# tuanad121/Python-WORLD

Measured on AMD Instinct MI355X. Metric: analysis+synthesis frames/sec (and xRT), 16 kHz / 5 ms hop, higher is better.
Workload: dtype f64; 1 GPU; BASELINE config 2 per GPU: 64 x 10 s synthetic 16 kHz utterances, DIO+StoneMask+CheapTrick+D4C encode + pulse-wise synthesis decode with on-device Philox noise (not the reference-parity host-noise path), HBM-resident; utterances_per_gpu=64, distinct_utterances=64, fs=16000, lanes_per_gpu=1

## Files before the change

include/world_hip.h:

```cpp
#ifndef WORLD_HIP_H
#define WORLD_HIP_H
#include <stddef.h>
#include <stdint.h>

#ifdef __cplusplus
extern "C" {
#endif

typedef struct wh_ctx wh_ctx;
typedef struct wh_batch wh_batch;

int wh_version(void);
const char* wh_last_error(void);

int wh_device_count(int* count);
int wh_ctx_create(int device, wh_ctx** out);
int wh_ctx_destroy(wh_ctx* ctx);
int wh_ctx_trim(wh_ctx* ctx);
int wh_malloc(void** dptr, size_t bytes);
int wh_free(void* dptr);
int wh_memcpy_h2d(void* dst, const void* h_src, size_t bytes, void* stream);
int wh_memcpy_d2h(void* h_dst, const void* src, size_t bytes, void* stream);
int wh_memset(void* dst, int value, size_t bytes, void* stream);
int wh_stream_sync(void* stream);
int wh_host_alloc(void** h_ptr, size_t bytes);
int wh_host_free(void* h_ptr);
int wh_copy_mapped(wh_ctx* ctx, void* stream, void* dst, const void* src, size_t bytes, int max_blocks);

#define WH_FLAG_STONEMASK_WINDOW 0
#define WH_FLAG_EVENT_OVERFLOW 1
#define WH_FLAG_NOISE_SHORT 2
#define WH_FLAG_NO_PULSE 3
#define WH_FLAG_PULSE_OVERFLOW 4
#define WH_FLAG_OOB 5
int wh_take_flags(wh_ctx* ctx, void* stream, int32_t* h_flags16);
int wh_bounds_build(void);
int wh_bounds_last(int64_t* out4);
int wh_bounds_selftest(wh_ctx* ctx, void* stream);
int wh_math_probe(wh_ctx* ctx, void* stream, int which, const double* in, double* out, int64_t n);
int wh_fft_probe(wh_ctx* ctx, void* stream, int n, int gt, int snt, int inverse, const double* in, double* out, int64_t count);
int wh_flags_post(wh_ctx* ctx, void* stream, int discard);
int wh_flags_poll(wh_ctx* ctx, int32_t* h_flags16);

int wh_profile_enable(wh_ctx* ctx, int on);
int wh_profile_collect(wh_ctx* ctx, char* names, size_t names_bytes, float* ms, int max_records, int* n_records);

int wh_batch_create(wh_ctx* ctx, int n_utt, const int64_t* h_x_off, const int64_t* h_frame_off, wh_batch** out);
int wh_batch_destroy(wh_batch* b);
int64_t wh_num_frames(int64_t n_samples, double fs, double frame_period_ms);

int wh_cheaptrick(wh_ctx* ctx, void* stream, const wh_batch* b, const double* x, const double* tp, double* f0,
                  const double* vuv, double fs, int fft_size, double q1, double* spectrogram, double* ps_spectrogram);

int wh_d4c(wh_ctx* ctx, void* stream, const wh_batch* b, const double* x, const double* tp, double* f0,
           const double* vuv, double fs, double threshold, int fft_size_for_spectrum, double* aperiodicity,
           double* coarse_ap);
int wh_d4c_bands(double fs, int requiem);

int wh_d4c_requiem(wh_ctx* ctx, void* stream, const wh_batch* b, const double* x, const double* tp, double* f0,
                   const double* vuv, double fs, double threshold, int fft_size, double* band_aperiodicity);

int wh_dio(wh_ctx* ctx, void* stream, const wh_batch* b, const double* x, const double* tp, double fs, double f0_floor,
           double f0_ceil, double target_fs, double frame_period_ms, double allowed_range, int n_bands,
           const double* h_band_f0, const int32_t* h_band_bias, const int32_t* h_band_len, const double* h_band_taps,
           const double* h_lowcut, int lowcut_half, double* f0_out, double* vuv_out, double* cand_out, double* raw_out);

int wh_harvest(wh_ctx* ctx, void* stream, const wh_batch* b, const double* x, const double* tp, double fs,
               double f0_floor, double f0_ceil, double frame_period_ms, int decimation_ratio, const double* h_ba,
               const double* h_zi, int n_bands, const double* h_band_f0, const int32_t* h_band_half,
               const double* h_band_taps, double* f0_out, double* vuv_out, double* dbg_y, double* dbg_raw,
               double* dbg_f0_1ms);
int wh_harvest_set_event_caps(wh_ctx* ctx, const int64_t* h_caps, int64_t n);
int wh_harvest_event_counts(wh_ctx* ctx, void* stream, int64_t* h_caps_out, int64_t n);
// ... 72 lines not shown
```

python-world_amd/csrc/wh_api.hip:

```cpp
#include <math.h>
#include <string.h>

#include "wh_device.h"
#include "wh_host.h"
#include "wh_math.h"

namespace {
thread_local std::string g_last_error;

__global__ void frame_utt_kernel(const int64_t* __restrict__ frame_off, int n_utt, int64_t total, int32_t* __restrict__ out) {
  int64_t i = (int64_t)blockIdx.x * blockDim.x + threadIdx.x;
  const int64_t stride = (int64_t)gridDim.x * blockDim.x;
  for (; i < total; i += stride) {
    int lo = 0, hi = n_utt;
    while (hi - lo > 1) {
      int mid = (lo + hi) >> 1;
      if (frame_off[mid] <= i) lo = mid; else hi = mid;
    }
    out[i] = lo;
  }
}

__global__ void copy_mapped_kernel(double2* __restrict__ dst, const double2* __restrict__ src, size_t n16, double* dst_tail,
                                   const double* src_tail) {
// ... 87 lines not shown
  e.host.assign(reinterpret_cast<const char*>(host), reinterpret_cast<const char*>(host) + bytes);
  *dptr = e.d;
  return 0;
}
int persistent_scratch(wh_ctx* ctx, const std::string& slot, size_t bytes, void** dptr) {
  wh_ctx::Persist& e = ctx->persist[slot];
  if (e.cap < bytes || !e.d) {
    if (e.d) {
      WH_CHECK(hipDeviceSynchronize());
      WH_CHECK(hipFree(e.d));
      e.d = nullptr;
    }
    const size_t want = bytes < 256 ? 256 : bytes + bytes / 4;
    WH_CHECK(hipMalloc(&e.d, want));
    e.cap = want;
  }
  *dptr = e.d;
  return 0;
}
}

static std::vector<int (*)(unsigned long long*)>& bounds_readers() {
  static std::vector<int (*)(unsigned long long*)> v;
  return v;
}
int wh::bounds_register(int (*reader)(unsigned long long*)) {
  bounds_readers().push_back(reader);
  return (int)bounds_readers().size();
}
static thread_local int64_t g_bounds_last[4] = {0, 0, 0, 0};

extern "C" {

int wh_version(void) { return 108; }
const char* wh_last_error(void) { return g_last_error.c_str(); }

int wh_device_count(int* count) {
  WH_CHECK(hipGetDeviceCount(count));
  return 0;
}

int wh_ctx_create(int device, wh_ctx** out) {
  if (!out) return wh::fail_msg("wh_ctx_create", "null out pointer");
  WH_CHECK(hipSetDevice(device));
  wh_ctx* c = new wh_ctx();
  c->device = device;
  std::vector<double2> tw(WH_TWIDDLE_ENTRIES);
  tw[0] = tw[1] = make_double2(1.0, 0.0);
  for (int n = 2; n <= WH_MAX_TWIDDLE; n <<= 1) {
    for (int k = 0; k < n; ++k) {
      long double a = -2.0L * 3.14159265358979323846264338327950288L * (long double)k / (long double)n;
      tw[n + k] = make_double2((double)cosl(a), (double)sinl(a));
    }
    tw[n] = make_double2(1.0, 0.0);
    if (n >= 2) tw[n + n / 2] = make_double2(-1.0, 0.0);
    if (n >= 4) {
      tw[n + n / 4] = make_double2(0.0, -1.0);
      tw[n + 3 * n / 4] = make_double2(0.0, 1.0);
    }
  }
  for (int R = 2; R <= 8; R <<= 1)
    for (int m = R; m <= WH_MAX_FFT; m <<= 1)
      for (int k = 0; k < m / R; ++k)
        for (int r = 1; r < R; ++r) tw[wh::fft_ptw_offset(m, R) + k * (R - 1) + r - 1] = tw[m + k * r];
  hipError_t e = hipMalloc((void**)&c->d_twiddle, tw.size() * sizeof(double2));
  if (e == hipSuccess) e = hipMemcpy(c->d_twiddle, tw.data(), tw.size() * sizeof(double2), hipMemcpyHostToDevice);
  if (e == hipSuccess) e = hipMalloc((void**)&c->d_flags, 16 * sizeof(int32_t));
// ... 114 lines not shown
  constexpr int N = 512;
  extern __shared__ __attribute__((aligned(16))) char smem[];
  const int g = threadIdx.x / GT, t = threadIdx.x % GT;
  const long long b = (long long)blockIdx.x * (SNT / GT) + g;
  const wh::ckp<double2> lds = wh::ck_make(reinterpret_cast<double2*>(smem), (long long)N * (SNT / GT), wh::WH_CK_LDS_OTHER);
  const wh::ckp<double2> s = wh::ck_sub(lds, (long long)g * N, N, wh::WH_CK_LDS_MAIN);
  const wh::ckp<const double2> tw = wh::ck_make(tw_base, WH_TWIDDLE_ENTRIES, wh::WH_CK_TWIDDLE);
  for (int i = t; i < N; i += GT) s[i] = b < count ? in[b * N + i] : make_double2(0.0, 0.0);
  __syncthreads();
  if (inv) wh::fft_lds_wave<N, true, GT, SNT>(s, tw + N);
  else wh::fft_lds_wave<N, false, GT, SNT>(s, tw + N);
  if (b < count)
    for (int i = t; i < N; i += GT) out[b * N + i] = s[i];
}
}
int wh_fft_probe(wh_ctx* ctx, void* stream, int n, int gt, int snt, int inverse, const double* in, double* out, int64_t count) {
  if (!ctx || !in || !out || count < 0 || n != 512 || (inverse != 0 && inverse != 1))
    return wh::fail_msg("wh_fft_probe", "bad argument");
  WH_ENTER(ctx);
  if (count == 0) return 0;
  const hipStream_t st = (hipStream_t)stream;
  const double2* a = reinterpret_cast<const double2*>(in);
  double2* o = reinterpret_cast<double2*>(out);
  auto launch = [&](auto kernel, int g, int t) {
    const int per = t / g;
    hipLaunchKernelGGL(kernel, dim3((unsigned)((count + per - 1) / per)), dim3(t), sizeof(double2) * 512 * per, st, a, o,
                       (const double2*)ctx->d_twiddle, (long long)count, inverse);
  };
  if (gt == 64 && snt == 64) launch(fft_probe_kernel<64, 64>, 64, 64);
  else if (gt == 128 && snt == 256) launch(fft_probe_kernel<128, 256>, 128, 256);
  else if (gt == 256 && snt == 256) launch(fft_probe_kernel<256, 256>, 256, 256);
  else return wh::fail_msg("wh_fft_probe", "shape not built (gt, snt): (64, 64), (128, 256), (256, 256)");
  WH_LAUNCH_CHECK("fft_probe_kernel");
  return 0;
}

int wh_bounds_last(int64_t* out4) {
  if (!out4) return wh::fail_msg("wh_bounds_last", "null argument");
  for (int i = 0; i < 4; ++i) out4[i] = g_bounds_last[i];
  return 0;
}

int wh_take_flags(wh_ctx* ctx, void* stream, int32_t* h_flags16) {
  if (!ctx || !h_flags16) return wh::fail_msg("wh_take_flags", "null argument");
  WH_ENTER(ctx);
  hipStream_t st = (hipStream_t)stream;
  WH_CHECK(hipMemcpyAsync(h_flags16, ctx->d_flags, 16 * sizeof(int32_t), hipMemcpyDeviceToHost, st));
  WH_CHECK(hipMemsetAsync(ctx->d_flags, 0, 16 * sizeof(int32_t), st));
  WH_CHECK(hipStreamSynchronize(st));
  drain_posted(ctx, h_flags16, true);
  for (int i = 0; i < 4; ++i) g_bounds_last[i] = 0;
  if (!bounds_readers().empty()) {
    WH_CHECK(hipDeviceSynchronize());
    for (auto rd : bounds_readers()) {
      unsigned long long rec[4] = {0, 0, 0, 0};
      if (rd(rec)) return wh::fail_msg("wh_take_flags", "reading a bounds record failed");
      if (rec[0]) {
        if (!g_bounds_last[0]) for (int i = 1; i < 4; ++i) g_bounds_last[i] = (int64_t)rec[i];
        g_bounds_last[0] += (int64_t)rec[0];
      }
    }
    if (g_bounds_last[0]) h_flags16[WH_FLAG_OOB] = 1;
  }
  return 0;
}

// ... 169 lines not shown
```

python-world_amd/csrc/wh_d4c.hip:

```cpp
#include <map>

#include <hip/hip_runtime.h>
#ifndef WH_D4C_PAIR
#define WH_D4C_PAIR 1
#endif
#ifndef WH_D4C_HOIST
#define WH_D4C_HOIST 0
#endif
#ifndef WH_D4C_PAIR_MINW
#define WH_D4C_PAIR_MINW 2
#endif
__device__ __forceinline__ int wh_opaque_tid() {
  int t = threadIdx.x;
#if !WH_D4C_HOIST
  asm volatile("" : "+v"(t));
#endif
  return t;
}
#define WH_TID wh_opaque_tid()
#include "wh_host.h"
#include "wh_spectral.h"

#ifndef WH_D4C_ABLATE
#define WH_D4C_ABLATE 0
#endif
#ifndef WH_D4C_KEEP_W
#define WH_D4C_KEEP_W 4
#endif
#ifndef WH_D4C_GATHER_UNCOND
#define WH_D4C_GATHER_UNCOND 1
#endif
#ifndef WH_D4C_REGFED
#define WH_D4C_REGFED 1
#endif
#ifndef WH_D4C_RMAXR
#define WH_D4C_RMAXR 0
#endif
#ifndef WH_D4C_MAXR
#define WH_D4C_MAXR 0
#endif
constexpr int d4c_maxr(int n) { return WH_D4C_MAXR ? WH_D4C_MAXR : ((n <= 1024 || WH_D4C_REGFED) ? 8 : 4); }
constexpr int d4c_rmaxr(int n) { return WH_D4C_RMAXR ? WH_D4C_RMAXR : ((n <= 1024 || WH_D4C_REGFED) ? 8 : 4); }
#ifndef WH_LOVE_REGWIN
#define WH_LOVE_REGWIN 1
#endif
#ifndef WH_LOVE_MAXR
#define WH_LOVE_MAXR 8
#endif
#ifndef WH_D4C_MINBLK
#define WH_D4C_MINBLK 4
#endif
#ifndef WH_D4C_WIN_UNROLL
#define WH_D4C_WIN_UNROLL 4
#endif
#ifndef WH_D4C_CENT_LOOP
#define WH_D4C_CENT_LOOP 0
#endif
#ifdef WH_D4C_STAGE_TIMER
__device__ unsigned long long g_d4c_stage[16];
__device__ unsigned long long g_d4c_t0[1 << 20];
#define STAGE_TIMER_BEGIN { if (threadIdx.x == 0) g_d4c_t0[blockIdx.x & ((1 << 20) - 1)] = __builtin_readcyclecounter(); }
#define STAGE_MARK(i) { __syncthreads(); if (threadIdx.x == 0) { const unsigned long long _t = __builtin_readcyclecounter(); atomicAdd(&g_d4c_stage[i], _t - g_d4c_t0[blockIdx.x & ((1 << 20) - 1)]); g_d4c_t0[blockIdx.x & ((1 << 20) - 1)] = _t; } }
#else
#define STAGE_TIMER_BEGIN
#define STAGE_MARK(i)
#endif
// ... 280 lines not shown
          if (!(j < L)) val = 0.0;
        } else {
          if (j < L) {
            const double w = shape(c);
            val = out[q] * w - w * dc;
            if (ENERGY) val *= inv_nrm;
          }
          const double cn = c * rot_c - sn * rot_s;
          sn = sn * rot_c + c * rot_s;
          c = cn;
        }
        out[q] = val;
      }
    }
  }
}
struct D4cLaunchConst {
  int b0, b1, b2;
  int boundary;
  int centre[8];
};
inline D4cLaunchConst d4c_launch_const(double fs, int n, int wlen, int interval, int nap) {
  D4cLaunchConst c;
  c.b0 = (int)(ceil(100.0 / (fs / n)) + 1);
  c.b1 = (int)(ceil(4000.0 / (fs / n)) + 1);
  c.b2 = (int)(ceil(7900.0 / (fs / n)) + 1);
  c.boundary = (int)((double)n / wlen * 8 + 0.5);
  for (int b = 0; b < 8; ++b) c.centre[b] = b < nap ? (int)floor((double)interval * (b + 1) / (fs / n)) : 0;
  return c;
}

template <int N>
constexpr bool d4c_regfed() { return WH_D4C_REGFED && N == 8 * ft_of(N); }

#ifndef WH_FT_LOVE_DIV
#define WH_FT_LOVE_DIV 2
#endif
constexpr int ft_love(int n) { return ft_of(n) / WH_FT_LOVE_DIV < 64 ? 64 : ft_of(n) / WH_FT_LOVE_DIV; }
template <int NLT>
__global__ __launch_bounds__(ft_love(NLT)) void love_train_kernel(
    const double* __restrict__ x, const int64_t* __restrict__ x_off, const int32_t* __restrict__ frame_utt,
    const double* __restrict__ tp, double* __restrict__ f0_io, const double* __restrict__ vuv, double fs,
    double threshold, const double2* __restrict__ tw_base, int32_t* __restrict__ gate, long long n_frames) {
  constexpr int FT = ft_love(NLT);
  extern __shared__ __attribute__((aligned(16))) char smem[];
  const wh::ckp<double> lds_all = wh::ck_make(reinterpret_cast<double*>(smem), NLT + 2 + 48 + kWinTab, wh::WH_CK_LDS_OTHER);
  const wh::ckp<double> zr = wh::ck_sub(lds_all, 0, NLT + 2, wh::WH_CK_LDS_MAIN);
  const wh::ckp<double2> zb = wh::ck_as<double2>(zr);
  const wh::ckp<double> scratch = wh::ck_sub(lds_all, NLT + 2, 48, wh::WH_CK_LDS_SCRATCH);
  const wh::ckp<double> wtab = wh::ck_sub(lds_all, NLT + 2 + 48, kWinTab, wh::WH_CK_LDS_AUX);
  const wh::ckp<const double2> tw = wh::ck_make(tw_base, WH_TWIDDLE_ENTRIES, wh::WH_CK_TWIDDLE);
  const int64_t f = wh::xcd_unit(blockIdx.x, n_frames);
  if (f >= n_frames) return;
  double f0 = f0_io[f];
  if (vuv[f] == 0.0) f0 = 0.0;
  if (threadIdx.x == 0) f0_io[f] = f0;
  if (f0 == 0.0) {
    if (threadIdx.x == 0) gate[f] = 0;
    return;
  }
  const int u = frame_utt[f];
  const long long xn = x_off[u + 1] - x_off[u];
  const wh::ckp<const double> xu = wh::ck_make(x + x_off[u], xn, wh::WH_CK_WAVEFORM);
  const double cf = fmax(f0, 40.0);
  if (threadIdx.x == 0) win_setup(wtab, xn, fs, cf, tp[f], 1.5, FT);
  wh::sync<FT>();
// ... 268 lines not shown
        const double y_hi = tmp[nlow - 1 - hi];
        const double slope = (y_hi - y_lo) / (a_hi - a_lo);
        inc = slope * (fk - a_lo) + y_lo;
      }
      add[kk] = inc;
    }
    if (one_wave) wh::sync<64>(); else wh::sync<FT>();
#pragma unroll
    for (int r = 0; r < KR; ++r) {
      const int kk = k0 + r;
      if (kk < nlow && nlow >= 2 && ((double)kk / N * fs) < f0) p[r] = add[kk] + p[r];
    }
  }
  wh::sync<FT>();
}

template <int N>
__device__ __forceinline__ void fill_mirrored_runs(const double (&p)[Runs<N>::KR], wh::ckp<double> v, double fs) {
  constexpr int FT = Runs<N>::FT, K = Runs<N>::K, KR = Runs<N>::KR;
  const int k0 = threadIdx.x * KR;
  const double df = fs / N;
#pragma unroll
  for (int r = 0; r < KR; ++r) {
    const int k = k0 + r;
    if (k < K) {
      const double val = p[r] * df;
      v[k] = val;
      if (k > 0 && k < N / 2) v[N - k] = val;
    }
  }
  wh::sync<FT>();
}

template <int N>
__device__ __forceinline__ void add_centroid(wh::ckp<const double> xu, wh::ckp<const double> wtab, double2 e_tid,
                                             wh::ckp<double2> buf, double (&cent)[Runs<N>::KR], bool first,
                                             wh::ckp<const double2> tw_base, wh::ckp<double> scratch) {
  constexpr int FT = Runs<N>::FT, K = Runs<N>::K, KR = Runs<N>::KR;
  if constexpr (d4c_regfed<N>()) {
    double val[N / FT];
    d4c_window_regs<true, N, true>(xu, wtab, e_tid, scratch, val);
    double2 zin[N / FT];
#pragma unroll
    for (int q = 0; q < N / FT; ++q) zin[q] = make_double2(val[q], val[q] * (double)(WH_TID + q * FT + 1));
    wh::fft_lds_from_regs<N, false, FT, 8>(zin, buf, fresh_table(tw_base) + N);
  } else {
    d4c_window<true, N, true, 2>(xu, wtab, e_tid, scratch, wh::ck_as<double>(buf),
                                 [&](int j, double val) { buf[j] = make_double2(val, val * (double)(j + 1)); });
    wh::sync<FT>();
    wh::fft_lds<N, false, FT, FT, d4c_maxr(N)>(buf, fresh_table(tw_base) + N);
  }
  const int k0 = threadIdx.x * KR;
#pragma unroll
  for (int r = 0; r < KR; ++r) {
    const int k = k0 + r;
    if (k < K) {
      const double2 a = buf[k];
      const double2 b = buf[(N - k) & (N - 1)];
      const double sr = 0.5 * (a.x + b.x), si = 0.5 * (a.y - b.y);
      const double tr = 0.5 * (a.y + b.y), ti = -0.5 * (a.x - b.x);
      const double c = tr * sr + si * ti;
      cent[r] = first ? c : cent[r] + c;
    }
  }
  wh::sync<FT>();
}

template <int N, bool FUSED>
__device__ __forceinline__ void d4c_frame(
    const double* __restrict__ x, const int64_t* __restrict__ x_off, const int32_t* __restrict__ frame_utt,
    const double* __restrict__ tp, double* __restrict__ f0_io, const double* __restrict__ vuv,
    const int32_t* __restrict__ gate, double threshold, double fs, int nap, int interval,
    const double* __restrict__ window, int wlen, const double2* __restrict__ tw_base,
    int k_spec,
    double* __restrict__ out, double* __restrict__ coarse_dbg, long long n_frames, const D4cLaunchConst& lc, int64_t f) {
  constexpr int FT = Runs<N>::FT, K = Runs<N>::K, KR = Runs<N>::KR;
  extern __shared__ __attribute__((aligned(16))) char smem[];
  const wh::ckp<double> lds_all = wh::ck_make(reinterpret_cast<double*>(smem), 2 * N + 40 + 8 + 4 * kWinTab, wh::WH_CK_LDS_OTHER);
  const wh::ckp<double> zr = wh::ck_sub(lds_all, 0, 2 * N, wh::WH_CK_LDS_MAIN);
  const wh::ckp<double2> buf = wh::ck_as<double2>(zr);
  const wh::ckp<double> scratch = wh::ck_sub(lds_all, 2 * N, 40, wh::WH_CK_LDS_SCRATCH);
  const wh::ckp<double> band = wh::ck_sub(lds_all, 2 * N + 40, 8, wh::WH_CK_LDS_AUX);
  const wh::ckp<double> wtab = wh::ck_sub(lds_all, 2 * N + 48, 4 * kWinTab, wh::WH_CK_LDS_AUX);
  constexpr int KPAD = (K + 1) & ~1;
  const wh::ckp<double> td = zr + (2 * N - KPAD);
  const wh::ckp<const double2> tw = wh::ck_make(tw_base, WH_TWIDDLE_ENTRIES, wh::WH_CK_TWIDDLE);
  const wh::ckp<const double> win_tab = wh::ck_make(window, wlen, wh::WH_CK_TABLE);

  STAGE_TIMER_BEGIN
  if (f >= n_frames) return;
  const int u = frame_utt[f];
  const long long xn = x_off[u + 1] - x_off[u];
  const wh::ckp<const double> xu = wh::ck_make(x + x_off[u], xn, wh::WH_CK_WAVEFORM);
  const double pos = tp[f];
  double f0v = f0_io[f];
  bool voiced;
  if (FUSED) {
    if (vuv[f] == 0.0) f0v = 0.0;
    if (threadIdx.x == 0) f0_io[f] = f0v;
    voiced = f0v != 0.0;
  } else {
    voiced = gate[f] != 0;
  }
  const double cf = fmax(47.0, f0v);
  const int k0 = threadIdx.x * KR;
  double pw[KR], cent[KR];
#pragma unroll
  for (int r = 0; r < KR; ++r) pw[r] = cent[r] = 0.0;
  if (voiced && threadIdx.x < 4) {
    const int wdx = threadIdx.x;
    const double wcf = wdx == 0 ? fmax(f0v, 40.0) : cf;
    const double wpos = wdx == 2 ? pos + 1 / cf / 4 : (wdx == 3 ? pos - 1 / cf / 4 : pos);
    win_setup(wtab + wdx * kWinTab, xn, fs, wcf, wpos, wdx == 0 ? 1.5 : 2.0, FT);
  }
  wh::sync<FT>();
  double2 e_frame = make_double2(0.0, 1.0);
// ... 34 lines not shown
          if (k < b1) s1 += pa;
        }
        const int km = N - k;
        if (k > 0 && k < N / 2 && km >= b0 && km < b2) {
          s2 += pa;
          if (km < b1) s1 += pa;
        }
      }
    }
    }
    wh::block_sum2<FT>(s1, s2, scratch);
    voiced = s1 / s2 > threshold;
  }
  if (!voiced) {
    if (k_spec > 0) {
      const wh::ckp<double> o = wh::ck_make(out + f * (int64_t)k_spec, k_spec, wh::WH_CK_OUT);
      for (int k = threadIdx.x; k < k_spec; k += FT) o[k] = 1 - 0.000000000001;
      if (coarse_dbg) for (int b = threadIdx.x; b < nap; b += FT) coarse_dbg[f * nap + b] = 0.0;
    } else {
      const wh::ckp<double> o = wh::ck_make(out + f * (int64_t)(nap + 2), nap + 2, wh::WH_CK_OUT);
      for (int b = threadIdx.x; b < nap + 2; b += FT) o[b] = -0.000000000001;
    }
    return;
  }

#if WH_D4C_ABLATE == 1
  if (threadIdx.x == 0) out[f * (int64_t)(k_spec > 0 ? k_spec : nap + 2)] = pw[0];
  return;
#endif
  STAGE_MARK(0)
#if WH_D4C_CENT_LOOP
#pragma unroll 1
  for (int c = 0; c < 2; ++c) {
    add_centroid<N>(xu, wtab + (2 + c) * kWinTab, e_frame, buf, cent, false, tw, scratch);
    STAGE_MARK(1 + c)
  }
#else
  add_centroid<N>(xu, wtab + 2 * kWinTab, e_frame, buf, cent, true, tw, scratch);
  STAGE_MARK(1)
  add_centroid<N>(xu, wtab + 3 * kWinTab, e_frame, buf, cent, false, tw, scratch);
  STAGE_MARK(2)
#endif
  low_band_replica_runs<N>(cent, zr, fs, cf, 1.2 * cf);
  STAGE_MARK(3)

#if WH_D4C_ABLATE == 2
  if (threadIdx.x == 0) out[f * (int64_t)(k_spec > 0 ? k_spec : nap + 2)] = cent[0] + pw[3];
  return;
#endif
  if (!FUSED) {
    d4c_window<false, N, false, 1>(xu, wtab + kWinTab, e_frame, scratch, zr, [&](int j, double val) { zr[j] = val; });
    wh::sync<FT>();
    wh::rfft_lds<N, FT, FT, d4c_rmaxr(N)>(buf, fresh_table(tw));
#pragma unroll
    for (int r = 0; r < KR; ++r) {
      if (k0 + r < K) {
        const double2 z = buf[k0 + r];
        pw[r] = z.x * z.x + z.y * z.y;
      }
    }
    wh::sync<FT>();
  }
  const wh::ckp<double> cum = zr;
  const double inv_cf = 1.0 / cf;
  low_band_replica_runs<N>(pw, cum, fs, cf, 1.2 * cf);
  double bandv[KR];
  wh::BandWindow bw;
  fill_mirrored_runs<N>(pw, cum, fs);
  bw.init(cum, N, fs, cf / 2);
  bw.run<KR>(k0, K, bandv);
#pragma unroll
  for (int r = 0; r < KR; ++r) cent[r] = cent[r] / (bandv[r] * inv_cf);
  wh::sync<FT>();
  fill_mirrored_runs<N>(cent, cum, fs);
  {
    const double w2 = cf / 2;
    const double inv_w2 = 1.0 / w2;
    bw.init(cum, N, fs, w2 / 2);
    bw.run<KR>(k0, K, bandv);
#pragma unroll
    for (int r = 0; r < KR; ++r) pw[r] = bandv[r] * inv_w2;
  }
  wh::sync<FT>();
  fill_mirrored_runs<N>(pw, cum, fs);
  bw.init(cum, N, fs, cf / 2);
  bw.run<KR>(k0, K, bandv);
  wh::sync<FT>();
#pragma unroll
  for (int r = 0; r < KR; ++r)
    if (k0 + r < K) td[k0 + r] = pw[r] - bandv[r] * inv_cf;
  wh::sync<FT>();

#if WH_D4C_ABLATE == 3
  if (threadIdx.x == 0) out[f * (int64_t)(k_spec > 0 ? k_spec : nap + 2)] = td[threadIdx.x];
  return;
#endif
  STAGE_MARK(4)
  const int boundary = lc.boundary;
  const int half = wlen / 2;
  constexpr int WQ = (N / 2 + 1 + FT - 1) / FT;
  double wv[WQ];
#pragma unroll
  for (int q = 0; q < WQ; ++q) {
    const int j = threadIdx.x + q * FT;
    wv[q] = win_tab[j < wlen ? j : 0];
  }
  for (int b = 0; b < nap; ++b) {
    const int centre = lc.centre[b];
#pragma unroll
    for (int q = 0; q < N / FT; ++q) {
      const int j = threadIdx.x + q * FT;
      double val = 0.0;
      if (j < wlen) {
        int idx = centre - half + j;
        idx = idx < 0 ? -idx : idx;
        idx = idx > N / 2 ? N - idx : idx;
        val = td[idx] * (q < WQ ? wv[q < WQ ? q : 0] : win_tab[j]);
      }
      zr[j] = val;
    }
    wh::sync<FT>();
    STAGE_MARK(12)
    constexpr int MB = N / 2;
    constexpr int PJ = (MB / 2 + 1 + FT - 1) / FT;
    double px[2 * PJ];
    unsigned pvalid = 0;
    {
      const wh::ckp<const double2> twb = fresh_table(tw);
      wh::fft_lds<MB, false, FT, FT, d4c_rmaxr(N)>(buf, twb + MB);
      const wh::ckp<const double2> WH_RESTRICT wpost = twb + N;
#pragma unroll
      for (int i = 0; i < PJ; ++i) {
        const int k = threadIdx.x + i * FT;
        px[2 * i] = px[2 * i + 1] = 0.0;
        if (k <= MB / 2) {
          const double2 a = buf[k], b = buf[MB - k];
          if (k == 0) {
            px[0] = (a.x + a.y) * (a.x + a.y);
            px[1] = (a.x - a.y) * (a.x - a.y);
            pvalid |= 3u;
          } else {
            const double er = 0.5 * (a.x + b.x), ei = 0.5 * (a.y - b.y);
            const double dr = 0.5 * (a.x - b.x), di = 0.5 * (a.y + b.y);
            const double2 wk = wh::ldg2(wpost + k);
            const double tr = fma(wk.x, di, wk.y * dr);
            const double ti = fma(wk.y, di, -(wk.x * dr));
            const double xr = er + tr, xi = ei + ti, yr = er - tr, yi = ti - ei;
            px[2 * i] = xr * xr + xi * xi;
            pvalid |= 1u << (2 * i);
            if (k != MB - k) {
              px[2 * i + 1] = yr * yr + yi * yi;
              pvalid |= 2u << (2 * i);
            }
          }
        }
      }
    }
    STAGE_MARK(13)
    wh::sync<FT>();
    STAGE_MARK(9)
    double s_small, s_total;
#if WH_D4C_ABLATE == 5
    s_small = px[0];
    s_total = px[1] + 1.0 + (double)pvalid;
#else
    sum_smallest<K, FT, 2 * PJ>(px, pvalid, N / 2 - boundary, zr, scratch, &s_small, &s_total);
#endif
    if (threadIdx.x == 0) band[b] = -10 * log10(s_small / s_total);
    wh::sync<FT>();
// ... 61 lines not shown
  }
#else
  d4c_frame<N, FUSED>(x, x_off, frame_utt, tp, f0_io, vuv, gate, threshold, fs, nap, interval, window, wlen, tw_base, k_spec, out,
                      coarse_dbg, n_frames, lc, wh::xcd_unit(blockIdx.x, n_frames));
#endif
}

int pow2_at_least(double v) { return (int)llround(pow(2.0, ceil(log2(v)))); }

std::vector<double> nuttall(int n) {
  std::vector<double> w(n);
  for (int i = 0; i < n; ++i) {
    const double t = (double)i * 2 * M_PI / (double)(n - 1);
    w[i] = 0.355768 * cos(0 * t) + -0.487396 * cos(t) + 0.144232 * cos(2 * t) + -0.012604 * cos(3 * t);
  }
  return w;
}

template <int NLT>
int launch_lt(wh_ctx* ctx, hipStream_t st, const wh_batch* b, const double* x, const double* tp, double* f0,
              const double* vuv, double fs, double thr, int32_t* gate) {
  const size_t lds = sizeof(double) * (NLT + 2 + 48 + kWinTab);
  if (int rc = wh::allow_lds(&love_train_kernel<NLT>, lds)) return rc;
  { wh::KernelTimer _kt(ctx, st, "love_train_kernel"); hipLaunchKernelGGL(love_train_kernel<NLT>, dim3((unsigned)wh::xcd_grid(b->total_frames)), dim3(ft_love(NLT)), lds, st, x, b->d_x_off,
                     b->d_frame_utt, tp, f0, vuv, fs, thr, ctx->d_twiddle, gate, (long long)b->total_frames); }
  WH_LAUNCH_CHECK("love_train_kernel");
  return 0;
}

template <int N, bool FUSED>
int launch_main(wh_ctx* ctx, hipStream_t st, const wh_batch* b, const double* x, const double* tp, double* f0,
                const double* vuv, const int32_t* gate, double thr, double fs, int nap, int interval, const double* win,
                int wlen, int k_spec, double* out, double* coarse) {
  const size_t lds = sizeof(double) * (2 * N + 40 + 8 + 4 * kWinTab);
  if (int rc = wh::allow_lds(&d4c_kernel<N, FUSED>, lds)) return rc;
  { wh::KernelTimer _kt(ctx, st, "d4c_kernel"); hipLaunchKernelGGL((d4c_kernel<N, FUSED>), dim3((unsigned)wh::xcd_grid((b->total_frames + WH_D4C_PAIR - 1) / WH_D4C_PAIR)), dim3(ft_of(N)), lds, st, x, b->d_x_off,
                     b->d_frame_utt, tp, f0, vuv, gate, thr, fs, nap, interval, win, wlen, ctx->d_twiddle, k_spec, out,
                     coarse, (long long)b->total_frames, d4c_launch_const(fs, N, wlen, interval, nap)); }
  WH_LAUNCH_CHECK("d4c_kernel");
  return 0;
}

int d4c_common(wh_ctx* ctx, void* stream, const wh_batch* b, const double* x, const double* tp, double* f0,
               const double* vuv, double fs, double threshold, int nfft, int interval, int k_spec, double* out,
               double* coarse) {
  hipStream_t st = (hipStream_t)stream;
  if (b->total_frames == 0) return 0;
  const int nap = (int)floor(fmin(15000.0, fs / 2 - interval) / interval);
  if (nap <= 0) return wh::fail_msg("wh_d4c", "sampling rate too low: no aperiodicity band (reference asserts, d4c.py:35)");
  if (nap > 8) return wh::fail_msg("wh_d4c", "more than 8 aperiodicity bands unsupported");
  const int nlt = pow2_at_least(3 * fs / 40.0 + 1);
  const int wlen = (int)(floor(interval / (fs / nfft)) * 2 + 1);
  if (int rc = wh::ws_reserve(ctx, (size_t)b->total_frames * sizeof(int32_t))) return rc;
  int32_t* gate = reinterpret_cast<int32_t*>(ctx->ws);
  const double* d_win = nullptr;
  if (int rc = wh::const_table(ctx, "nuttall:" + std::to_string(wlen), nuttall(wlen), &d_win)) return rc;
  if (nlt == nfft) {
    switch (nfft) {
      case 512: return launch_main<512, true>(ctx, st, b, x, tp, f0, vuv, gate, threshold, fs, nap, interval, d_win, wlen, k_spec, out, coarse);
      case 1024: return launch_main<1024, true>(ctx, st, b, x, tp, f0, vuv, gate, threshold, fs, nap, interval, d_win, wlen, k_spec, out, coarse);
      case 2048: return launch_main<2048, true>(ctx, st, b, x, tp, f0, vuv, gate, threshold, fs, nap, interval, d_win, wlen, k_spec, out, coarse);
      case 4096: return launch_main<4096, true>(ctx, st, b, x, tp, f0, vuv, gate, threshold, fs, nap, interval, d_win, wlen, k_spec, out, coarse);
      case 8192: return launch_main<8192, true>(ctx, st, b, x, tp, f0, vuv, gate, threshold, fs, nap, interval, d_win, wlen, k_spec, out, coarse);
      default: return wh::fail_msg("wh_d4c", "D4C FFT size outside [512, 8192]");
    }
  }
  int rc;
// ... 58 lines not shown
```

python-world_amd/csrc/wh_device.h:

```cpp
#pragma once
#include <hip/hip_runtime.h>
#include <stdint.h>

#define WH_BLOCK 256
#define WH_WAVE 64
#ifndef WH_TID
#define WH_TID threadIdx.x
#endif

#define WH_MAX_FFT 8192
#define WH_MAX_TWIDDLE 32768

namespace wh {

__device__ __forceinline__ double2 ldg2(const double2* p) {
  typedef double v2d __attribute__((ext_vector_type(2)));
  const v2d v = *(const v2d __attribute__((address_space(1)))*)p;
  return make_double2(v.x, v.y);
}
__device__ __forceinline__ double ldg(const double* p) { return *(const double __attribute__((address_space(1)))*)p; }
#if WH_BOUNDS
template <class T> struct ckp;
__device__ __forceinline__ double2 ldg2(const ckp<const double2>& p);
__device__ __forceinline__ double ldg(const ckp<const double>& p);
// ... 450 lines not shown
    constexpr bool SWZ = WH_FFT_SWZ && N >= 64 && MAXR >= 8;
    fft_pass<N, NT, R, NS, INV, SNT, SWZ && (NS > 1), SWZ && (NS * R < N)>(s, tw);
    fft_passes<N, NT, NS * R, INV, SNT, MAXR>(s, tw);
  }
}

template <int N, bool INV, int NT = WH_BLOCK, int SNT = NT, int MAXR = 8>
__device__ __forceinline__ void fft_lds(ckp<double2> s, ckp<const double2> tw) {
  fft_passes<N, NT, 1, INV, SNT, MAXR>(s, tw);
}

#define WH_HAVE_FFT_WAVE 1
template <int N, bool INV, int GT, int SNT = GT>
__device__ __forceinline__ void fft_lds_wave(ckp<double2> s, ckp<const double2> tw) {
  static_assert(N / 8 <= WH_WAVE && GT % WH_WAVE == 0 && SNT % GT == 0, "one wave must own a pass's butterflies");
  if ((WH_TID & (GT - 1)) < WH_WAVE) fft_lds<N, INV, WH_WAVE, WH_WAVE>(s, tw);
  sync_lds<SNT>();
}

template <int N, bool INV, int NT = WH_BLOCK, int MAXR = 8>
__device__ __forceinline__ void fft_lds_from_regs(const double2 (&x)[N / NT], ckp<double2> s, ckp<const double2> tw) {
  constexpr int R = FftRadix<N, NT, 1, MAXR>::value;
  static_assert(N % (R * NT) == 0 && N >= 64, "register-fed first pass needs N >= R*NT");
  constexpr int PER = N / R / NT;
  double2 v[PER][R], w[PER][R];
#pragma unroll
  for (int p = 0; p < PER; ++p)
#pragma unroll
    for (int r = 0; r < R; ++r) v[p][r] = x[p + r * PER];
  sync_lds<NT>();
  fft_pass_finish<N, NT, R, 1, INV, (WH_FFT_SWZ && R < N && MAXR >= 8)>(s, v, w);
  sync_lds<NT>();
  fft_passes<N, NT, R, INV, NT, MAXR>(s, tw);
}


template <int N, int NT = WH_BLOCK, int SNT = NT, int MAXR = 8>
__device__ __forceinline__ void rfft_lds(ckp<double2> z, ckp<const double2> WH_RESTRICT tw_base) {
  fft_lds<N / 2, false, NT, SNT, MAXR>(z, tw_base + N / 2);
  ckp<const double2> WH_RESTRICT w = tw_base + N;
  for (int k = WH_TID & (NT - 1); k <= N / 4; k += NT) {
    if (k == 0) {
      const double2 a = z[0];
      z[0] = make_double2(a.x + a.y, 0.0);
      z[N / 2] = make_double2(a.x - a.y, 0.0);
    } else {
      const double2 a = z[k], b = z[N / 2 - k];
      const double er = 0.5 * (a.x + b.x), ei = 0.5 * (a.y - b.y);
      const double dr = 0.5 * (a.x - b.x), di = 0.5 * (a.y + b.y);
      const double2 wk = ldg2(w + k);
      const double tr = fma(wk.x, di, wk.y * dr);
      const double ti = fma(wk.y, di, -(wk.x * dr));
      z[k] = make_double2(er + tr, ei + ti);
      z[N / 2 - k] = make_double2(er - tr, ti - ei);
    }
  }
  sync_lds<SNT>();
}

template <int N, int NT = WH_BLOCK, int SNT = NT, int MAXR = 8>
__device__ __forceinline__ void irfft_lds(ckp<double2> z, ckp<const double2> WH_RESTRICT tw_base) {
  ckp<const double2> WH_RESTRICT w = tw_base + N;
  for (int k = WH_TID & (NT - 1); k <= N / 4; k += NT) {
    double2 a = z[k], b = z[N / 2 - k];
    if (k == 0) {
      a.y = 0.0;
// ... 16 lines not shown
```

python-world_amd/world/_hip.py:

```python
import contextlib
import ctypes
import os
import threading

import numpy as np

_HERE = os.path.dirname(os.path.abspath(__file__))
LIB_PATH = os.environ.get("WH_LIB") or os.path.join(os.path.dirname(_HERE), "lib", "libworld_hip.so")

_c_i64p = ctypes.POINTER(ctypes.c_int64)
_vp = ctypes.c_void_p
_dbl = ctypes.c_double
_int = ctypes.c_int

SIGNATURES = {
    "wh_version": (_int, []),
    "wh_last_error": (ctypes.c_char_p, []),
    "wh_device_count": (_int, [ctypes.POINTER(_int)]),
    "wh_ctx_create": (_int, [_int, ctypes.POINTER(_vp)]),
    "wh_ctx_destroy": (_int, [_vp]),
    "wh_ctx_trim": (_int, [_vp]),
    "wh_malloc": (_int, [ctypes.POINTER(_vp), ctypes.c_size_t]),
    "wh_free": (_int, [_vp]),
    "wh_memcpy_h2d": (_int, [_vp, _vp, ctypes.c_size_t, _vp]),
    "wh_memcpy_d2h": (_int, [_vp, _vp, ctypes.c_size_t, _vp]),
    "wh_memset": (_int, [_vp, _int, ctypes.c_size_t, _vp]),
    "wh_stream_sync": (_int, [_vp]),
    "wh_host_alloc": (_int, [ctypes.POINTER(_vp), ctypes.c_size_t]),
    "wh_host_free": (_int, [_vp]),
    "wh_copy_mapped": (_int, [_vp, _vp, _vp, _vp, ctypes.c_size_t, _int]),
    "wh_batch_create": (_int, [_vp, _int, _c_i64p, _c_i64p, ctypes.POINTER(_vp)]),
    "wh_batch_destroy": (_int, [_vp]),
    "wh_num_frames": (ctypes.c_int64, [ctypes.c_int64, _dbl, _dbl]),
    "wh_cheaptrick": (_int, [_vp, _vp, _vp, _vp, _vp, _vp, _vp, _dbl, _int, _dbl, _vp, _vp]),
    "wh_profile_enable": (_int, [_vp, _int]),
    "wh_profile_collect": (_int, [_vp, ctypes.c_char_p, ctypes.c_size_t, ctypes.POINTER(ctypes.c_float), _int,
                                  ctypes.POINTER(_int)]),
    "wh_take_flags": (_int, [_vp, _vp, ctypes.POINTER(ctypes.c_int32)]),
    "wh_bounds_build": (_int, []),
    "wh_bounds_last": (_int, [_c_i64p]),
    "wh_bounds_selftest": (_int, [_vp, _vp]),
    "wh_math_probe": (_int, [_vp, _vp, _int, _vp, _vp, ctypes.c_int64]),
    "wh_fft_probe": (_int, [_vp, _vp, _int, _int, _int, _int, _vp, _vp, ctypes.c_int64]),
    "wh_flags_post": (_int, [_vp, _vp, _int]),
    "wh_flags_poll": (_int, [_vp, ctypes.POINTER(ctypes.c_int32)]),
    "wh_dio": (_int, [_vp, _vp, _vp, _vp, _vp, _dbl, _dbl, _dbl, _dbl, _dbl, _dbl, _int, _vp, _vp, _vp, _vp, _vp, _int,
                      _vp, _vp, _vp, _vp]),
    "wh_harvest": (_int, [_vp, _vp, _vp, _vp, _vp, _dbl, _dbl, _dbl, _dbl, _int, _vp, _vp, _int, _vp, _vp, _vp, _vp, _vp,
                          _vp, _vp, _vp]),
    "wh_harvest_set_event_caps": (_int, [_vp, _vp, ctypes.c_int64]),
    "wh_harvest_event_counts": (_int, [_vp, _vp, _vp, ctypes.c_int64]),
    "wh_stonemask": (_int, [_vp, _vp, _vp, _vp, _vp, _vp, _dbl, _vp, _int, _vp]),
    "wh_synthesis": (_int, [_vp, _vp, _vp, _vp, _vp, _vp, _vp, _vp, _dbl, _int, _vp, _vp, _vp, ctypes.c_int64, _vp, _vp,
                            ctypes.c_uint64, _vp, _vp]),
    "wh_synthesis_timebase": (_int, [_vp, _vp, _vp, _vp, _vp, _vp, _dbl, _vp, _vp, _vp, ctypes.c_int64, _dbl]),
    "wh_synthesis_render": (_int, [_vp, _vp, _vp, _vp, _vp, _vp, _vp, _dbl, _int, _vp, _vp, _vp, ctypes.c_int64, _vp, _vp,
                                   ctypes.c_uint64, _vp, _vp]),
    "wh_philox_normals": (_int, [_vp, _vp, ctypes.c_uint64, _int, ctypes.c_int64, ctypes.c_int64, _vp]),
    "wh_cumsum_exact": (_int, [_vp, _vp, _vp, _vp, _int]),
    "wh_peak_normalise": (_int, [_vp, _vp, _vp, _vp, _int]),
    "wh_synthesis_plan": (_int, [_vp, _vp, _vp, _vp, _vp, _vp, _dbl, _vp, _vp, _vp, ctypes.c_int64, _vp, _vp]),
    "wh_synthesis_requiem": (_int, [_vp, _vp, _vp, _vp, _vp, _vp, _vp, _vp, _dbl, _int, _vp, _vp, _vp, _vp, ctypes.c_int64,
                                    _vp, _int, _vp, ctypes.c_int64, _int, _vp, _vp]),
    "wh_d4c": (_int, [_vp, _vp, _vp, _vp, _vp, _vp, _vp, _dbl, _dbl, _int, _vp, _vp]),
    "wh_d4c_bands": (_int, [_dbl, _int]),
    "wh_d4c_requiem": (_int, [_vp, _vp, _vp, _vp, _vp, _vp, _vp, _dbl, _dbl, _int, _vp]),
    "wh_feature_matmul": (_int, [_vp, _vp, _vp, ctypes.c_int64, _int, ctypes.c_int64, _int, _vp, _dbl, _vp, _int, _int, _vp,
                                 ctypes.c_int64]),
    "wh_feature_matmul_tagged": (_int, [_vp, _vp, _vp, ctypes.c_int64, _int, ctypes.c_int64, _int, _vp, _dbl, _vp, _int, _int,
                                        _vp, ctypes.c_int64, ctypes.c_uint64]),
    "wh_context_frames": (_int, [_vp, _vp, _vp, ctypes.c_int64, _int, _int, _vp]),
    "wh_warp_spectrum": (_int, [_vp, _vp, _vp, ctypes.c_int64, _int, _vp, _vp, _vp]),
    "wh_modify_duration": (_int, [_vp, _vp, _vp, _vp, _vp, _vp, _vp, _int]),
    "wh_pcm16_to_f64": (_int, [_vp, _vp, _vp, ctypes.c_int64, _vp]),
    "wh_f64_to_pcm16": (_int, [_vp, _vp, _vp, ctypes.c_int64, _vp]),
    "wh_swipe": (_int, [_vp, _vp, _vp, _vp, _dbl, _dbl, _dbl, _int, _vp, _int, _int, _vp, _vp, _vp, _vp, _int, _vp, _vp]),
# ... 294 lines not shown
```

Measured before the change: 14.15 million frames/s.

## Use two-level register-fed FFT with padded LDS layout in fused D4C kernel

Adds a two-level FFT in which each thread first does a radix-R1 butterfly in registers, then independent sub-FFTs run per wave on a padded LDS layout with strided bin indexing. The fused D4C kernel with N=2048 uses it for both centroid FFTs and the per-band half-size FFT, feeding band samples from registers as packed real pairs instead of writing them to LDS and syncing first. The aim is fewer LDS passes and block-wide barriers per transform. In exchange, LDS usage grows slightly from padding, bin reads are now strided, and a probe entry point is added for testing.

Result: no change. 14.23 million frames/s (median of 6 runs) (+0.5%).

```diff
diff --git a/include/world_hip.h b/include/world_hip.h
--- a/include/world_hip.h
+++ b/include/world_hip.h
@@ -39,6 +39,7 @@
 int wh_bounds_selftest(wh_ctx* ctx, void* stream);
 int wh_math_probe(wh_ctx* ctx, void* stream, int which, const double* in, double* out, int64_t n);
 int wh_fft_probe(wh_ctx* ctx, void* stream, int n, int gt, int snt, int inverse, const double* in, double* out, int64_t count);
+int wh_fft2l_probe(wh_ctx* ctx, void* stream, int n, int r1, int maxr, const double* in, double* out, int64_t count);
 int wh_flags_post(wh_ctx* ctx, void* stream, int discard);
 int wh_flags_poll(wh_ctx* ctx, int32_t* h_flags16);
 
diff --git a/python-world_amd/csrc/wh_api.hip b/python-world_amd/csrc/wh_api.hip
--- a/python-world_amd/csrc/wh_api.hip
+++ b/python-world_amd/csrc/wh_api.hip
@@ -143,7 +143,7 @@
 
 extern "C" {
 
-int wh_version(void) { return 108; }
+int wh_version(void) { return 109; }
 const char* wh_last_error(void) { return g_last_error.c_str(); }
 
 int wh_device_count(int* count) {
@@ -324,6 +324,43 @@
   else if (gt == 256 && snt == 256) launch(fft_probe_kernel<256, 256>, 256, 256);
   else return wh::fail_msg("wh_fft_probe", "shape not built (gt, snt): (64, 64), (128, 256), (256, 256)");
   WH_LAUNCH_CHECK("fft_probe_kernel");
+  return 0;
+}
+
+extern "C++" {
+template <int N, int R1, int MAXR2>
+static __global__ __launch_bounds__(256) void fft2l_probe_kernel(const double2* __restrict__ in, double2* __restrict__ out,
+                                                                const double2* __restrict__ tw_base, long long count) {
+  using L = wh::Fft2l<N, R1>;
+  extern __shared__ __attribute__((aligned(16))) char smem[];
+  const long long b = blockIdx.x;
+  const wh::ckp<double2> s = wh::ck_make(reinterpret_cast<double2*>(smem), (long long)L::SPAN, wh::WH_CK_LDS_MAIN);
+  const wh::ckp<const double2> tw = wh::ck_make(tw_base, WH_TWIDDLE_ENTRIES, wh::WH_CK_TWIDDLE);
+  double2 x[R1];
+#pragma unroll
+  for (int r = 0; r < R1; ++r) x[r] = in[b * N + threadIdx.x + r * (N / R1)];
+  wh::fft2l_from_regs<N, 256, R1, MAXR2>(x, s, tw + N);
+  for (int k = threadIdx.x; k < N; k += 256) out[b * N + k] = s[L::index(k)];
+}
+}
+int wh_fft2l_probe(wh_ctx* ctx, void* stream, int n, int r1, int maxr, const double* in, double* out, int64_t count) {
+  if (!ctx || !in || !out || count < 0 || count > 0x7fffffff || (maxr != 4 && maxr != 8))
+    return wh::fail_msg("wh_fft2l_probe", "bad argument");
+  WH_ENTER(ctx);
+  const hipStream_t st = (hipStream_t)stream;
+  const double2* a = reinterpret_cast<const double2*>(in);
+  double2* o = reinterpret_cast<double2*>(out);
+  auto launch = [&](auto kernel, int span) {
+    if (count > 0)
+      hipLaunchKernelGGL(kernel, dim3((unsigned)count), dim3(256), sizeof(double2) * span, st, a, o,
+                         (const double2*)ctx->d_twiddle, (long long)count);
+  };
+  if (n == 2048 && r1 == 8 && maxr == 8) launch(fft2l_probe_kernel<2048, 8, 8>, wh::Fft2l<2048, 8>::SPAN);
+  else if (n == 2048 && r1 == 8) launch(fft2l_probe_kernel<2048, 8, 4>, wh::Fft2l<2048, 8>::SPAN);
+  else if (n == 1024 && r1 == 4 && maxr == 8) launch(fft2l_probe_kernel<1024, 4, 8>, wh::Fft2l<1024, 4>::SPAN);
+  else if (n == 1024 && r1 == 4) launch(fft2l_probe_kernel<1024, 4, 4>, wh::Fft2l<1024, 4>::SPAN);
+  else return wh::fail_msg("wh_fft2l_probe", "shape not built (n, r1): (2048, 8), (1024, 4)");
+  WH_LAUNCH_CHECK("fft2l_probe_kernel");
   return 0;
 }
 
diff --git a/python-world_amd/csrc/wh_d4c.hip b/python-world_amd/csrc/wh_d4c.hip
--- a/python-world_amd/csrc/wh_d4c.hip
+++ b/python-world_amd/csrc/wh_d4c.hip
@@ -32,6 +32,9 @@
 #endif
 #ifndef WH_D4C_REGFED
 #define WH_D4C_REGFED 1
+#endif
+#ifndef WH_D4C_BAND_MAXR2
+#define WH_D4C_BAND_MAXR2 4
 #endif
 #ifndef WH_D4C_RMAXR
 #define WH_D4C_RMAXR 0
@@ -378,6 +381,12 @@
 
 template <int N>
 constexpr bool d4c_regfed() { return WH_D4C_REGFED && N == 8 * ft_of(N); }
+template <int N, bool FUSED>
+constexpr bool d4c_twolevel() { return FUSED && N == 2048 && d4c_regfed<N>(); }
+template <int N, bool FUSED>
+constexpr int d4c_zr_doubles() {
+  return d4c_twolevel<N, FUSED>() && 2 * wh::Fft2l<N, 8>::SPAN > 2 * N ? 2 * wh::Fft2l<N, 8>::SPAN : 2 * N;
+}
 
 #ifndef WH_FT_LOVE_DIV
 #define WH_FT_LOVE_DIV 2
@@ -712,7 +721,7 @@
   wh::sync<FT>();
 }
 
-template <int N>
+template <int N, bool TL>
 __device__ __forceinline__ void add_centroid(wh::ckp<const double> xu, wh::ckp<const double> wtab, double2 e_tid,
                                              wh::ckp<double2> buf, double (&cent)[Runs<N>::KR], bool first,
                                              wh::ckp<const double2> tw_base, wh::ckp<double> scratch) {
@@ -723,7 +732,8 @@
     double2 zin[N / FT];
 #pragma unroll
     for (int q = 0; q < N / FT; ++q) zin[q] = make_double2(val[q], val[q] * (double)(WH_TID + q * FT + 1));
-    wh::fft_lds_from_regs<N, false, FT, 8>(zin, buf, fresh_table(tw_base) + N);
+    if constexpr (TL) wh::fft2l_from_regs<N, FT, 8>(zin, buf, fresh_table(tw_base) + N);
+    else wh::fft_lds_from_regs<N, false, FT, 8>(zin, buf, fresh_table(tw_base) + N);
   } else {
     d4c_window<true, N, true, 2>(xu, wtab, e_tid, scratch, wh::ck_as<double>(buf),
                                  [&](int j, double val) { buf[j] = make_double2(val, val * (double)(j + 1)); });
@@ -731,12 +741,13 @@
     wh::fft_lds<N, false, FT, FT, d4c_maxr(N)>(buf, fresh_table(tw_base) + N);
   }
   const int k0 = threadIdx.x * KR;
+  auto bin = [](int k) { return TL ? wh::Fft2l<N, 8>::index(k) : k; };
 #pragma unroll
   for (int r = 0; r < KR; ++r) {
     const int k = k0 + r;
     if (k < K) {
-      const double2 a = buf[k];
-      const double2 b = buf[(N - k) & (N - 1)];
+      const double2 a = buf[bin(k)];
+      const double2 b = buf[bin((N - k) & (N - 1))];
       const double sr = 0.5 * (a.x + b.x), si = 0.5 * (a.y - b.y);
       const double tr = 0.5 * (a.y + b.y), ti = -0.5 * (a.x - b.x);
       const double c = tr * sr + si * ti;
@@ -755,13 +766,15 @@
     int k_spec,
     double* __restrict__ out, double* __restrict__ coarse_dbg, long long n_frames, const D4cLaunchConst& lc, int64_t f) {
   constexpr int FT = Runs<N>::FT, K = Runs<N>::K, KR = Runs<N>::KR;
+  constexpr bool TL = d4c_twolevel<N, FUSED>();
+  constexpr int ZR = d4c_zr_doubles<N, FUSED>();
   extern __shared__ __attribute__((aligned(16))) char smem[];
-  const wh::ckp<double> lds_all = wh::ck_make(reinterpret_cast<double*>(smem), 2 * N + 40 + 8 + 4 * kWinTab, wh::WH_CK_LDS_OTHER);
-  const wh::ckp<double> zr = wh::ck_sub(lds_all, 0, 2 * N, wh::WH_CK_LDS_MAIN);
+  const wh::ckp<double> lds_all = wh::ck_make(reinterpret_cast<double*>(smem), ZR + 40 + 8 + 4 * kWinTab, wh::WH_CK_LDS_OTHER);
+  const wh::ckp<double> zr = wh::ck_sub(lds_all, 0, ZR, wh::WH_CK_LDS_MAIN);
   const wh::ckp<double2> buf = wh::ck_as<double2>(zr);
-  const wh::ckp<double> scratch = wh::ck_sub(lds_all, 2 * N, 40, wh::WH_CK_LDS_SCRATCH);
-  const wh::ckp<double> band = wh::ck_sub(lds_all, 2 * N + 40, 8, wh::WH_CK_LDS_AUX);
-  const wh::ckp<double> wtab = wh::ck_sub(lds_all, 2 * N + 48, 4 * kWinTab, wh::WH_CK_LDS_AUX);
+  const wh::ckp<double> scratch = wh::ck_sub(lds_all, ZR, 40, wh::WH_CK_LDS_SCRATCH);
+  const wh::ckp<double> band = wh::ck_sub(lds_all, ZR + 40, 8, wh::WH_CK_LDS_AUX);
+  const wh::ckp<double> wtab = wh::ck_sub(lds_all, ZR + 48, 4 * kWinTab, wh::WH_CK_LDS_AUX);
   constexpr int KPAD = (K + 1) & ~1;
   const wh::ckp<double> td = zr + (2 * N - KPAD);
   const wh::ckp<const double2> tw = wh::ck_make(tw_base, WH_TWIDDLE_ENTRIES, wh::WH_CK_TWIDDLE);
@@ -862,13 +875,13 @@
 #if WH_D4C_CENT_LOOP
 #pragma unroll 1
   for (int c = 0; c < 2; ++c) {
-    add_centroid<N>(xu, wtab + (2 + c) * kWinTab, e_frame, buf, cent, false, tw, scratch);
+    add_centroid<N, TL>(xu, wtab + (2 + c) * kWinTab, e_frame, buf, cent, false, tw, scratch);
     STAGE_MARK(1 + c)
   }
 #else
-  add_centroid<N>(xu, wtab + 2 * kWinTab, e_frame, buf, cent, true, tw, scratch);
+  add_centroid<N, TL>(xu, wtab + 2 * kWinTab, e_frame, buf, cent, true, tw, scratch);
   STAGE_MARK(1)
-  add_centroid<N>(xu, wtab + 3 * kWinTab, e_frame, buf, cent, false, tw, scratch);
+  add_centroid<N, TL>(xu, wtab + 3 * kWinTab, e_frame, buf, cent, false, tw, scratch);
   STAGE_MARK(2)
 #endif
   low_band_replica_runs<N>(cent, zr, fs, cf, 1.2 * cf);
@@ -928,43 +941,58 @@
   STAGE_MARK(4)
   const int boundary = lc.boundary;
   const int half = wlen / 2;
-  constexpr int WQ = (N / 2 + 1 + FT - 1) / FT;
+  constexpr int WQ = TL ? 2 * ((N / 2 + 1) / (2 * FT)) : (N / 2 + 1 + FT - 1) / FT;
   double wv[WQ];
 #pragma unroll
   for (int q = 0; q < WQ; ++q) {
-    const int j = threadIdx.x + q * FT;
+    const int j = TL ? 2 * threadIdx.x + (q >> 1) * 2 * FT + (q & 1) : threadIdx.x + q * FT;
     wv[q] = win_tab[j < wlen ? j : 0];
   }
+  constexpr int MB = N / 2;
   for (int b = 0; b < nap; ++b) {
     const int centre = lc.centre[b];
-#pragma unroll
-    for (int q = 0; q < N / FT; ++q) {
-      const int j = threadIdx.x + q * FT;
-      double val = 0.0;
-      if (j < wlen) {
-        int idx = centre - half + j;
-        idx = idx < 0 ? -idx : idx;
-        idx = idx > N / 2 ? N - idx : idx;
-        val = td[idx] * (q < WQ ? wv[q < WQ ? q : 0] : win_tab[j]);
-      }
-      zr[j] = val;
-    }
-    wh::sync<FT>();
+    auto tap_sample = [&](int j, double w) {
+      int idx = centre - half + j;
+      idx = idx < 0 ? -idx : idx;
+      idx = idx > N / 2 ? N - idx : idx;
+      return td[idx] * w;
+    };
+    double2 zin[TL ? MB / FT : 1];
+    if constexpr (TL) {
+#pragma unroll
+      for (int r = 0; r < MB / FT; ++r) {
+        double val[2];
+#pragma unroll
+        for (int e = 0; e < 2; ++e) {
+          const int q = 2 * r + e, j = 2 * (int)threadIdx.x + r * 2 * FT + e;
+          val[e] = j < wlen ? tap_sample(j, q < WQ ? wv[q < WQ ? q : 0] : win_tab[j]) : 0.0;
+        }
+        zin[r] = make_double2(val[0], val[1]);
+      }
+    } else {
+#pragma unroll
+      for (int q = 0; q < N / FT; ++q) {
+        const int j = threadIdx.x + q * FT;
+        zr[j] = j < wlen ? tap_sample(j, q < WQ ? wv[q < WQ ? q : 0] : win_tab[j]) : 0.0;
+      }
+      wh::sync<FT>();
+    }
     STAGE_MARK(12)
-    constexpr int MB = N / 2;
     constexpr int PJ = (MB / 2 + 1 + FT - 1) / FT;
     double px[2 * PJ];
     unsigned pvalid = 0;
     {
       const wh::ckp<const double2> twb = fresh_table(tw);
-      wh::fft_lds<MB, false, FT, FT, d4c_rmaxr(N)>(buf, twb + MB);
+      if constexpr (TL) wh::fft2l_from_regs<MB, FT, MB / FT, WH_D4C_BAND_MAXR2>(zin, buf, twb + MB);
+      else wh::fft_lds<MB, false, FT, FT, d4c_rmaxr(N)>(buf, twb + MB);
+      auto bin = [](int k) { return TL ? wh::Fft2l<MB, MB / FT>::index(k & (MB - 1)) : k; };
       const wh::ckp<const double2> WH_RESTRICT wpost = twb + N;
 #pragma unroll
       for (int i = 0; i < PJ; ++i) {
         const int k = threadIdx.x + i * FT;
         px[2 * i] = px[2 * i + 1] = 0.0;
         if (k <= MB / 2) {
-          const double2 a = buf[k], b = buf[MB - k];
+          const double2 a = buf[bin(k)], b = buf[bin(MB - k)];
           if (k == 0) {
             px[0] = (a.x + a.y) * (a.x + a.y);
             px[1] = (a.x - a.y) * (a.x - a.y);
@@ -1092,7 +1120,7 @@
 int launch_main(wh_ctx* ctx, hipStream_t st, const wh_batch* b, const double* x, const double* tp, double* f0,
                 const double* vuv, const int32_t* gate, double thr, double fs, int nap, int interval, const double* win,
                 int wlen, int k_spec, double* out, double* coarse) {
-  const size_t lds = sizeof(double) * (2 * N + 40 + 8 + 4 * kWinTab);
+  const size_t lds = sizeof(double) * (d4c_zr_doubles<N, FUSED>() + 40 + 8 + 4 * kWinTab);
   if (int rc = wh::allow_lds(&d4c_kernel<N, FUSED>, lds)) return rc;
   { wh::KernelTimer _kt(ctx, st, "d4c_kernel"); hipLaunchKernelGGL((d4c_kernel<N, FUSED>), dim3((unsigned)wh::xcd_grid((b->total_frames + WH_D4C_PAIR - 1) / WH_D4C_PAIR)), dim3(ft_of(N)), lds, st, x, b->d_x_off,
                      b->d_frame_utt, tp, f0, vuv, gate, thr, fs, nap, interval, win, wlen, ctx->d_twiddle, k_spec, out,
diff --git a/python-world_amd/csrc/wh_device.h b/python-world_amd/csrc/wh_device.h
--- a/python-world_amd/csrc/wh_device.h
+++ b/python-world_amd/csrc/wh_device.h
@@ -506,6 +506,38 @@
   fft_pass_finish<N, NT, R, 1, INV, (WH_FFT_SWZ && R < N && MAXR >= 8)>(s, v, w);
   sync_lds<NT>();
   fft_passes<N, NT, R, INV, NT, MAXR>(s, tw);
+}
+
+#define WH_HAVE_FFT2L 1
+template <int N, int R1>
+struct Fft2l {
+  static constexpr int M = N / R1;
+  static constexpr int PAD = R1 == 8 ? 14 : 4;
+  static constexpr int PITCH = M + PAD;
+  static constexpr int SPAN = (R1 - 1) * PITCH + M;
+  __device__ static __forceinline__ int index(int k) { return (k & (R1 - 1)) * PITCH + k / R1; }
+};
+template <int N, int NT, int R1, int MAXR2 = 8>
+__device__ __forceinline__ void fft2l_from_regs(const double2 (&x)[R1], ckp<double2> s, ckp<const double2> tw) {
+  using L = Fft2l<N, R1>;
+  constexpr int M = L::M, NW = NT / WH_WAVE, SPW = R1 / NW, ST = WH_WAVE / SPW;
+  static_assert(M == NT && NT % WH_WAVE == 0 && R1 % NW == 0 && SPW * ST == WH_WAVE, "shape of the two-level transform");
+  const int n = WH_TID & (NT - 1);
+  const ckp<const double2> pt = tw + (fft_ptw_offset(N, R1) - N);
+  double2 v[R1], w[R1];
+#pragma unroll
+  for (int r = 1; r < R1; ++r) w[r] = ldg2(pt + (n * (R1 - 1) + r - 1));
+#pragma unroll
+  for (int r = 0; r < R1; ++r) v[r] = x[r];
+  sync_lds<NT>();
+  dft_small<R1, false>(v);
+  s[n] = v[0];
+#pragma unroll
+  for (int r = 1; r < R1; ++r) s[r * L::PITCH + n] = cmul(v[r], w[r]);
+  sync_lds<NT>();
+  const int sub = ((WH_TID & (NT - 1)) >> 6) * SPW + (WH_TID & (WH_WAVE - 1)) / ST;
+  fft_lds<M, false, ST, WH_WAVE, MAXR2>(s + sub * L::PITCH, tw - (N - M));
+  sync_lds<NT>();
 }
 
 
diff --git a/python-world_amd/world/_hip.py b/python-world_amd/world/_hip.py
--- a/python-world_amd/world/_hip.py
+++ b/python-world_amd/world/_hip.py
@@ -42,6 +42,7 @@
     "wh_bounds_selftest": (_int, [_vp, _vp]),
     "wh_math_probe": (_int, [_vp, _vp, _int, _vp, _vp, ctypes.c_int64]),
     "wh_fft_probe": (_int, [_vp, _vp, _int, _int, _int, _int, _vp, _vp, ctypes.c_int64]),
+    "wh_fft2l_probe": (_int, [_vp, _vp, _int, _int, _int, _vp, _vp, ctypes.c_int64]),
     "wh_flags_post": (_int, [_vp, _vp, _int]),
     "wh_flags_poll": (_int, [_vp, ctypes.POINTER(ctypes.c_int32)]),
     "wh_dio": (_int, [_vp, _vp, _vp, _vp, _vp, _dbl, _dbl, _dbl, _dbl, _dbl, _dbl, _int, _vp, _vp, _vp, _vp, _vp, _int,
```
